# austintheriot/ray-tracer-webgl

Hardware: AMD Instinct MI355X
Metric: Mray/s (ray segments/s) at 1920x1080 (higher is better)
Workload: dtype f32

## Files before the change

ray_tracer_webgl_amd/csrc/pt_api.hip:

```cpp
#include <hip/hip_runtime.h>

#include <mutex>
#include <chrono>
#include <cmath>
#include <cstdarg>
#include <cstdio>
#include <cstdlib>
#include <cstring>
#include <new>
#include <string>
#include <thread>
#include <utility>
#include <vector>

#include "../../include/ptrace.h"
#include "../../include/ptrace_dev.h"
#include "pt_bvh.hpp"
#include "pt_grid.hpp"
#include "pt_grid_records.hpp"
#include "pt_scene_image.hpp"
#include "pt_extra.h"
#include "pt_sigs.h"
#include "pt_kernel_args.h"
#include "pt_geom_plan.hpp"
// ... 231 lines not shown
  }
  if (const ptbuf::Fit f = c->feat.fit(e); !f.ok()) return fit_refused(c, "feature planes", f, e);
  {
    if (c->query.on && !c->query.fits(e)) PT_HIP(c, hipStreamSynchronize(c->stream));
    const ptbuf::Fit f = c->query.fit(e);
    if (f.fresh & c->query.ORDER) PT_HIP(c, fill_identity_order(c->query.order, e.tiles));
    if (!f.ok()) return fit_refused(c, "query planes", f, e);
  }
  if (const ptbuf::Fit f = c->hist.fit(e); !f.ok()) return fit_refused(c, "history planes", f, e);
  {
    const ptbuf::Fit f = c->expo.fit();
    if (f.fresh & c->expo.STATE) PT_HIP(c, zero(c->expo.state, c->expo.kWords));
    if (!f.ok()) return fit_refused(c, "exposure state", f, e);
  }
  if (const ptbuf::Fit f = c->glare.fit(c->width, c->local_rows); !f.ok()) return fit_refused(c, "glare pyramid", f, e);
  return PT_OK;
}

int frame_buffers_ready(pt_ctx* c, const char* who) {
  const ptbuf::Extent e = extent_of(c);
  if (c->frame.in_place(e) && (!c->est.on || c->est.in_place(e, c->hist.on))) return PT_OK;
  return fail(c, PT_ERR_CAPACITY, "%s: the context's buffers are not allocated for the rows in place (an earlier allocation failed)", who);
}

enum OptInSet { SET_ESTIMATE, SET_FEATURES, SET_QUERIES, SET_REPROJECT, SET_TONEMAP, SET_GLARE, SET_NEXT_EVENT };
int option_off(pt_ctx* c, const char* who, OptInSet set, int code = PT_ERR_NOT_READY) {
  static const char* const what[] = {"the error estimate is off (pt_set_option PT_OPT_ERROR_ESTIMATE)", "the feature planes are off (pt_set_option PT_OPT_FEATURES)",
                                     "ray queries are off (pt_set_option PT_OPT_RAY_QUERIES)", "reprojection is off (pt_set_option PT_OPT_REPROJECT)",
                                     "tone mapping is off (pt_set_option PT_OPT_TONEMAP)", "the glare is off (pt_set_option PT_OPT_GLARE)",
                                     "next-event estimation is off (pt_set_option PT_OPT_NEXT_EVENT)"};
  return fail(c, code, "%s: %s", who, what[set]);
}

int clear_error(pt_ctx* c) {
  if (!c->est.on) return PT_OK;
  const size_t pix = n_pixels(c);
  if (pix) PT_HIP(c, hipMemsetAsync(c->est.state.get(), 0, 2 * pix * sizeof(float4), c->stream));
  c->est.spp = 0;
  return PT_OK;
}

int empty_accum(pt_ctx* c) {
  const size_t pix = n_pixels(c);
  if (c->frame.accum && pix) PT_HIP(c, hipMemsetAsync(c->frame.accum, 0, pix * sizeof(float4), c->stream));
  return clear_error(c);
}

int fold_events(pt_ctx* c) {
  for (size_t i = 0; i < c->events_used; i++) {
    float ms = 0.f;
    PT_HIP(c, hipEventElapsedTime(&ms, c->events[i].first, c->events[i].second));
    c->kernel_ms += (double)ms;
  }
  c->events_used = 0;
  return PT_OK;
}

int next_events(pt_ctx* c, std::pair<hipEvent_t, hipEvent_t>** ev) {
  if (c->events_used == c->events.size()) {
    if (c->events.size() >= 512) {
      PT_HIP(c, hipStreamSynchronize(c->stream));
      int rc = fold_events(c);
      if (rc != PT_OK) return rc;
    } else {
      hipEvent_t a, b;
      PT_HIP(c, hipEventCreate(&a));
      PT_HIP(c, hipEventCreate(&b));
      c->events.emplace_back(a, b);
    }
  }
  *ev = &c->events[c->events_used++];
  return PT_OK;
}

struct TimedSpan {
  std::pair<hipEvent_t, hipEvent_t>* ev = nullptr;
  int take(pt_ctx* c) { return next_events(c, &ev); }
  int begin(pt_ctx* c) const {
    if (ev) PT_HIP(c, hipEventRecord(ev->first, c->stream));
    return PT_OK;
  }
  int end(pt_ctx* c) const {
    if (ev) PT_HIP(c, hipEventRecord(ev->second, c->stream));
    return PT_OK;
  }
};

bool is_capturing(const pt_ctx* c) {
  hipStreamCaptureStatus cap = hipStreamCaptureStatusNone;
  (void)hipStreamIsCapturing(c->stream, &cap);
  return cap != hipStreamCaptureStatusNone;
}
int not_capturing(pt_ctx* c, const char* who) {
  return is_capturing(c) ? fail(c, PT_ERR_INVALID, "%s: synchronises; not inside a stream capture", who) : PT_OK;
}

int scene_and_uniforms(pt_ctx* c, const char* who) {
  if (c->state.have_spheres && c->state.have_params) return PT_OK;
  return fail(c, PT_ERR_NOT_READY, "%s: pt_set_spheres and pt_set_params must come first", who);
}

int launch_tile_order(pt_ctx* c) {
  hipLaunchKernelGGL(pt_tile_order_kernel, dim3(1), dim3(1024), 0, c->stream, c->frame.tile_cost.get(), c->frame.tile_order.get(),
                     n_tiles(c));
  PT_HIP(c, hipGetLastError());
  return PT_OK;
}

void try_finish_tuning(pt_ctx* c) {
  if (!c->geom.awaiting_times()) return;
  for (int k = 0; k < c->geom.n_paths; k++)
    if (hipEventQuery(c->trial_ev[2 * k + 1]) != hipSuccess) return;
  double ms[4];
  for (int k = 0; k < c->geom.n_paths; k++) {
    float t = 0.f;
    if (hipEventElapsedTime(&t, c->trial_ev[2 * k], c->trial_ev[2 * k + 1]) != hipSuccess) return;
    ms[k] = (double)t;
  }
  c->geom.settle(ms);
}

PathScene path_scene(const pt_ctx* c) {
  return {c->list.n, c->bvh.present, c->grid.present, c->grid.head.max_cell_entries, c->grid.head.n_always};
}

double need_factor(const pt_ctx* c) {
  return c->grid.present && c->state.have_params ? view_need_factor(c->params, c->grid.head.c0, c->grid.head.s0) : 0.0;
}

int fit_state(const pt_ctx* c) {
  return grid_fit_state(c->geom.grid_in_use(c->grid.present), need_factor(c), (double)c->grid.head.near_factor);
}

Staging grid_build(const pt_ctx* c) {
  const ptgrid::Grid& g = c->grid.head;
  return grid_staging(ptscene::staged_cells(g), g.n_entries, walk_lds_room(), c->state.grid_cells_build, fit_state(c));
}

const void* cell_kernel(int device, const TraceCell& k) {
#define PT_TRACE_ACCESSOR_OF(object, accessor, n_ids) accessor,
  static const void* (*const accessors[OBJ_COUNT + 2])(int) = {PT_TRACE_OBJECTS(PT_TRACE_ACCESSOR_OF) pt_nee_kernel, pt_rad_nee_kernel};
  static_assert(OBJ_NEE == OBJ_COUNT && OBJ_RAD_NEE == OBJ_COUNT + 1, "the next-event objects follow the trace table's");
  static std::once_flag once[64][OBJ_COUNT + 2][PT_EXTRA_COUNT];
  static_assert(PT_EXTRA_COUNT >= PT_VARIANT_COUNT, "the extra object has the most ids");
  const void* fn = accessors[k.object](k.id);
  if (fn && k.object >= OBJ_EXTRA)
    std::call_once(once[device & 63][k.object][k.id], [fn] {
      (void)hipFuncSetAttribute(fn, hipFuncAttributeMaxDynamicSharedMemorySize, (int)kWalkLdsMax);
      (void)hipGetLastError();
    });
  return fn;
}

}

PT_API int pt_device_count(void) {
  int n = 0;
  if (hipGetDeviceCount(&n) != hipSuccess) return 0;
  return n;
}

PT_API const char* pt_last_error(pt_ctx* ctx) {
  return ctx ? ctx->error.c_str() : g_create_error.c_str();
}

static int create_common(pt_ctx** out, int device, uint32_t width, uint32_t height, void* caller_stream) {
  if (!out) return fail(nullptr, PT_ERR_INVALID, "pt_create: out is NULL");
  *out = nullptr;
  if (width == 0 || height == 0) return fail(nullptr, PT_ERR_INVALID, "pt_create: empty image");
  int n = 0;
  const double t_begin = host_ms();
  if (hipGetDeviceCount(&n) != hipSuccess || n <= 0)
    return fail(nullptr, PT_ERR_NO_DEVICE,
                "pt_create: no HIP device (libptrace has no CPU backend by design)");
  const double t_runtime = host_ms();
  if (device < 0 || device >= n)
    return fail(nullptr, PT_ERR_NO_DEVICE, "pt_create: device %d out of range (0..%d)", device, n - 1);
  pt_ctx* c = new (std::nothrow) pt_ctx();
  if (!c) return fail(nullptr, PT_ERR_INVALID, "pt_create: out of host memory");
  c->device = device;
  c->width = width;
  c->height = height;
  c->local_rows = height;
  auto bail = [&](hipError_t e, const char* what) {
    fail(nullptr, PT_ERR_HIP, "pt_create: %s: %s", what, hipGetErrorString(e));
    delete c;
    return PT_ERR_HIP;
  };
  hipError_t e;
  if ((e = hipSetDevice(device)) != hipSuccess) return bail(e, "hipSetDevice");
  hipDeviceProp_t prop;
  if ((e = hipGetDeviceProperties(&prop, device)) != hipSuccess) return bail(e, "hipGetDeviceProperties");
  c->num_cus = prop.multiProcessorCount > 0 ? prop.multiProcessorCount : 256;
  const double t_device = host_ms();
  if (caller_stream) {
    c->stream = (hipStream_t)caller_stream;
  } else {
    if ((e = hipStreamCreateWithFlags(&c->own_stream, hipStreamNonBlocking)) != hipSuccess)
      return bail(e, "hipStreamCreateWithFlags");
    c->stream = c->own_stream;
  }
  const double t_stream = host_ms();
  if ((e = (hipError_t)c->d_counters.reserve(PT_CTR_ALLOC)) != hipSuccess) return bail(e, "hipMalloc(counters)");
  const double t_first_malloc = host_ms();
  if ((e = hipMemsetAsync(c->d_counters.get(), 0, PT_CTR_ALLOC * sizeof(unsigned long long), c->stream)) != hipSuccess)
    return bail(e, "hipMemsetAsync(counters)");
  const double t_first_memset = host_ms();
  if ((e = (hipError_t)c->d_frame_ctr.reserve(2)) != hipSuccess) return bail(e, "hipMalloc(frame counter)");
  if ((e = hipMemsetAsync(c->d_frame_ctr.get(), 0, 2 * sizeof(uint32_t), c->stream)) != hipSuccess)
    return bail(e, "hipMemsetAsync(frame counter)");
  const double t_small_allocs = host_ms();
  for (int id = 0; id < PT_MAIN_COUNT; id++) (void)hipFuncSetAttribute(pt_main_kernel(id), hipFuncAttributeMaxDynamicSharedMemorySize, (int)kWalkLdsMax);
  (void)hipGetLastError();
  const double t_code = host_ms();
  int rc = ensure_buffers(c);
  if (rc != PT_OK) { g_create_error = c->error; delete c; return rc; }
  const double t_end = host_ms();
  c->setup_ms[PT_SETUP_CREATE_RUNTIME] = t_runtime - t_begin;
  c->setup_ms[PT_SETUP_CREATE_DEVICE] = t_device - t_runtime;
  c->setup_ms[PT_SETUP_CREATE_STREAM_ALLOCS] = t_small_allocs - t_device;
  c->setup_ms[PT_SETUP_CREATE_STREAM] = t_stream - t_device;
  c->setup_ms[PT_SETUP_CREATE_FIRST_MALLOC] = t_first_malloc - t_stream;
  c->setup_ms[PT_SETUP_CREATE_FIRST_MEMSET] = t_first_memset - t_first_malloc;
  c->setup_ms[PT_SETUP_CREATE_CODE_OBJECT] = t_code - t_small_allocs;
  c->setup_ms[PT_SETUP_CREATE_BUFFERS] = t_end - t_code;
  c->setup_ms[PT_SETUP_CREATE_TOTAL] = t_end - t_begin;
  *out = c;
  return PT_OK;
}

PT_API int pt_create(pt_ctx** out, int device, uint32_t width, uint32_t height) {
  return create_common(out, device, width, height, nullptr);
}
PT_API int pt_create_on_stream(pt_ctx** out, int device, uint32_t width, uint32_t height, void* hip_stream) {
  return create_common(out, device, width, height, hip_stream);
}

PT_API int pt_destroy(pt_ctx* c) {
  if (!c) return PT_ERR_INVALID;
  (void)hipSetDevice(c->device);
  (void)hipStreamSynchronize(c->stream);
  delete c;
  return PT_OK;
}

PT_API int pt_set_stream(pt_ctx* c, void* hip_stream) {
  if (!c) return PT_ERR_INVALID;
  PT_HIP(c, hipSetDevice(c->device));
  PT_HIP(c, hipStreamSynchronize(c->stream));
  int rc = fold_events(c);
  if (rc != PT_OK) return rc;
  if (!hip_stream && !c->own_stream)
    PT_HIP(c, hipStreamCreateWithFlags(&c->own_stream, hipStreamNonBlocking));
  c->stream = hip_stream ? (hipStream_t)hip_stream : c->own_stream;
  return PT_OK;
}

namespace {

#define PT_TRY(call) do { if (int rc_ = (call); rc_ != PT_OK) return rc_; } while (0)

template <class T>
int upload(pt_ctx* c, DevBuf<T>& buf, const T* src, size_t n, size_t n_pad, int pad_byte) {
  if (buf.capacity() < n_pad) PT_HIP(c, buf.reserve(n_pad));
  if (n_pad > n) PT_HIP(c, hipMemset(buf.get() + n, pad_byte, (n_pad - n) * sizeof(T)));
  if (n) PT_HIP(c, hipMemcpy(buf.get(), src, n * sizeof(T), hipMemcpyHostToDevice));
  return PT_OK;
}
template <class T>
int upload(pt_ctx* c, DevBuf<T>& buf, const std::vector<T>& src) { return upload(c, buf, src.data(), src.size(), src.size(), 0); }
template <class T>
void release(std::vector<T>& v) { std::vector<T>().swap(v); }

void drop_scene(pt_ctx* c) {
  c->bvh.present = c->grid.present = false;
  changed(*c, ptstate::SCENE_DROPPED);
}

int install_list(pt_ctx* c, const ptscene::Split& sp, size_t n) {
  PT_TRY(upload(c, c->list.geom, sp.geom));
  PT_TRY(upload(c, c->list.mat, sp.mat.data(), n, n ? n : 1u, 0));
  return upload(c, c->list.r0, sp.r0.data(), 2 * n, n ? 2 * n : 2u, 0);
}

int install_slots(pt_ctx* c, SceneSlots& s, const std::vector<uint32_t>& index, size_t n, size_t n_pad, const ptscene::Split& sp) {
  s.present = false;
  PT_TRY(upload(c, s.index, index.data(), n, n_pad, 0xff));
  s.index_n = n_pad;
  return upload(c, s.mat, ptscene::per_slot(index.data(), n, sp.mat.data(), sp.mat.size()).data(), n, n_pad, 0);
}

int install_bvh(pt_ctx* c, ptbvh::Bvh& bvh, const ptscene::Split& sp) {
  PT_TRY(install_slots(c, c->bvh, bvh.slot_index, bvh.slot_index.size(), bvh.slot_index.size(), sp));
  PT_TRY(upload(c, c->bvh.nodes, bvh.nodes16));
  PT_TRY(upload(c, c->bvh.nodes32, bvh.nodes32));
  PT_TRY(upload(c, c->bvh.slots, bvh.slots));
  release(bvh.nodes); release(bvh.nodes16); release(bvh.nodes32); release(bvh.slots); release(bvh.slot_index);
  c->bvh.head = std::move(bvh);
  c->bvh.present = true;
  return PT_OK;
}
int install_grid(pt_ctx* c, ptgrid::Grid& grid, const ptscene::Split& sp) {
  const size_t n_ent = grid.n_entries, n_ent_pad = n_ent + 4u;
  PT_TRY(install_slots(c, c->grid, grid.entry_index, n_ent, n_ent_pad, sp));
  PT_TRY(upload(c, c->grid.entries, grid.entries.data(), n_ent * 4, n_ent_pad * 4, 0));
  std::vector<uint32_t> recs(grid.cells.size());
  for (size_t k = 0; k < recs.size(); k++) recs[k] = ptrec::from_host(grid.cells[k]);
  PT_TRY(upload(c, c->grid.cells, recs.data(), recs.size(), (recs.size() + 3u) & ~(size_t)3u, 0));
  if (grid.n[1] == 1u) {
    recs.assign(((size_t)ptrec::ring_cells(grid.n[0], grid.n[2]) + 3u) & ~(size_t)3u, ptrec::kOutside);
    ptrec::ring_layout(grid.cells.data(), grid.n[0], grid.n[2], recs.data());
    PT_TRY(upload(c, c->grid.ring, recs));
  }
  release(grid.cells); release(grid.entries); release(grid.entry_index);
  c->grid.head = std::move(grid);
  c->grid.present = true;
  return PT_OK;
}

inline bool wants_uuids(const pt_ctx* c) { return c->dbg_enable || c->feat.on || c->query.on; }
int upload_uuids(pt_ctx* c, const std::vector<int32_t>& uuid) {
  PT_HIP(c, hipSetDevice(c->device));
  PT_HIP(c, hipStreamSynchronize(c->stream));
  PT_TRY(upload(c, c->list.uuid, uuid.data(), uuid.size(), uuid.empty() ? 1u : uuid.size(), 0));
  for (SceneSlots* s : std::initializer_list<SceneSlots*>{&c->bvh, &c->grid}) {
    if (!s->present || !s->index_n) continue;
    std::vector<uint32_t> index(s->index_n);
    PT_HIP(c, hipMemcpy(index.data(), s->index.get(), index.size() * sizeof(uint32_t), hipMemcpyDeviceToHost));
    PT_TRY(upload(c, s->uuid, ptscene::per_slot(index.data(), index.size(), uuid.data(), uuid.size())));
  }
  changed(*c, ptstate::UUIDS_UPLOADED);
  return PT_OK;
}

int upload_lights(pt_ctx* c, const ptscene::Split& sp, uint32_t n) {
  std::vector<ptnee::Light> table(n ? n : 1u);
  const uint32_t L = ptnee::lights_of(sp.geom.data(), sp.mat.data(), n, table.data());
  const ptbuf::Fit f = c->lights.fit(L);
  if (!f.ok()) return fail(c, PT_ERR_HIP, "PT_OPT_NEXT_EVENT: no room for the table of %u lights (%s)", L, hipGetErrorString((hipError_t)f.err));
  if (L) PT_HIP(c, hipMemcpy(c->lights.table.get(), table.data(), (size_t)L * sizeof(ptnee::Light), hipMemcpyHostToDevice));
  return PT_OK;
}

int install_scene(pt_ctx* c, const ptscene::Split& sp, uint32_t n, ptbvh::Bvh* bvh, ptgrid::Grid* grid) {
  PT_TRY(install_list(c, sp, n));
  if (bvh) PT_TRY(install_bvh(c, *bvh, sp));
  if (grid) PT_TRY(install_grid(c, *grid, sp));
  if (c->lights.on) PT_TRY(upload_lights(c, sp, n));
  return wants_uuids(c) ? upload_uuids(c, sp.uuid) : PT_OK;
}

}

PT_API int pt_set_spheres(pt_ctx* c, const PtSphere* s, uint32_t n) {
  if (!c || (!s && n)) return fail(c, PT_ERR_INVALID, "pt_set_spheres: NULL argument");
  if (n > PT_MAX_SPHERES)
    return fail(c, PT_ERR_CAPACITY, "pt_set_spheres: %u spheres exceed the 16-bit candidate index range (%u)",
                n, PT_MAX_SPHERES);
  PT_HIP(c, hipSetDevice(c->device));
  const double t_begin = host_ms();
  ptscene::Split sp = ptscene::split(s, n);
  const double t_split = host_ms();
  ptbvh::Bvh bvh;
  const bool have_bvh = sp.regular && ptbvh::build(sp.geom.data(), sp.radii.data(), n, &bvh);
  const double t_bvh = host_ms();
  ptgrid::Grid grid;
  const bool have_grid = sp.regular && ptscene::build_grid(sp.geom.data(), sp.radii.data(), n, 3.0, &grid);
  const double t_grid = host_ms();
  PT_HIP(c, hipStreamSynchronize(c->stream));
  drop_scene(c);
  if (int rc = install_scene(c, sp, n, have_bvh ? &bvh : nullptr, have_grid ? &grid : nullptr); rc != PT_OK) return drop_scene(c), rc;
  c->list.n = n;
  c->list.host = std::move(sp);
  changed(*c, ptstate::SCENE_INSTALLED);
  c->geom.reset();
  c->geom.list_paths(path_scene(c));
  const double t_end = host_ms();
  c->setup_ms[PT_SETUP_SPHERES_SPLIT] = t_split - t_begin;
  c->setup_ms[PT_SETUP_SPHERES_BVH_BUILD] = t_bvh - t_split;
  c->setup_ms[PT_SETUP_SPHERES_GRID_BUILD] = t_grid - t_bvh;
  c->setup_ms[PT_SETUP_SPHERES_UPLOAD] = t_end - t_grid;
  c->setup_ms[PT_SETUP_SPHERES_TOTAL] = t_end - t_begin;
  return PT_OK;
}

PT_API int pt_set_params(pt_ctx* c, const PtParams* p) {
  if (!c || !p) return fail(c, PT_ERR_INVALID, "pt_set_params: NULL argument");
  if (p->width != c->width || p->height != c->height)
    return fail(c, PT_ERR_INVALID, "pt_set_params: %ux%u does not match the context's %ux%u (use pt_resize)",
                p->width, p->height, c->width, c->height);
  if (p->samples_per_pixel < 1 || p->max_depth < 1)
    return fail(c, PT_ERR_INVALID, "pt_set_params: samples_per_pixel and max_depth must be >= 1");
  if (p->band_count > 1 && (p->band_rows == 0 || p->band_index >= p->band_count))
    return fail(c, PT_ERR_INVALID, "pt_set_params: bad row partition (rows %u index %u count %u)",
                p->band_rows, p->band_index, p->band_count);
  PT_HIP(c, hipSetDevice(c->device));
  uint32_t rows = count_local_rows(c->height, *p);
  const bool repartition = rows != c->local_rows || ptstate::Partition(*p) != ptstate::Partition(c->params);
  if (repartition && c->frame.accum_bound && (size_t)rows * c->width > c->frame.accum_pixels)
    return fail(c, PT_ERR_CAPACITY, "pt_set_params: bound accumulation buffer too small for %u rows", rows);
  if (repartition) {
    changed(*c, ptstate::ROWS_ASKED);
    const uint32_t old_rows = c->local_rows;
    c->local_rows = rows;
    int rc = ensure_buffers(c);
    if (rc != PT_OK) {
      c->local_rows = old_rows;
      return rc;
    }
    c->params = *p;
    changed(*c, ptstate::UNIFORMS_OTHER_ROWS);
    c->tally.repartitioned();
    if (int rc = empty_accum(c); rc != PT_OK) return rc;
    return pt_clear_textures(c);
  }
  c->params = *p;
  changed(*c, ptstate::UNIFORMS_SAME_ROWS);
  return PT_OK;
}

PT_API int pt_resize(pt_ctx* c, uint32_t width, uint32_t height) {
  if (!c || width == 0 || height == 0) return fail(c, PT_ERR_INVALID, "pt_resize: bad size");
  PT_HIP(c, hipSetDevice(c->device));
  PT_HIP(c, hipStreamSynchronize(c->stream));
  c->width = width;
  c->height = height;
  changed(*c, ptstate::RESIZED);
  c->params.band_count = 0;
  c->local_rows = height;
  if (c->frame.accum_bound) { c->frame.accum_bound = false; c->frame.accum = nullptr; }
  int rc = ensure_buffers(c);
  if (rc != PT_OK) return rc;
  rc = pt_clear_textures(c);
  if (rc != PT_OK) return rc;
  return pt_reset_accum(c);
}

PT_API int pt_reserve_passes(pt_ctx* c, uint32_t max_passes) {
  if (!c || max_passes == 0) return fail(c, PT_ERR_INVALID, "pt_reserve_passes: bad argument");
  PT_HIP(c, hipSetDevice(c->device));
  const double t_begin = host_ms();
  const uint32_t reserved = c->reserved_passes;
  if (max_passes > reserved) {
    PT_HIP(c, hipStreamSynchronize(c->stream));
    c->reserved_passes = max_passes;
  }
  const int rc = ensure_buffers(c);
  if (rc != PT_OK) c->reserved_passes = reserved;
  c->setup_ms[PT_SETUP_RESERVE_TOTAL] = host_ms() - t_begin;
  return rc;
}

PT_API int pt_reset_accum(pt_ctx* c) {
  if (!c) return PT_ERR_INVALID;
  PT_HIP(c, hipSetDevice(c->device));
  PT_HIP(c, hipMemsetAsync(c->d_counters.get(), 0, PT_CTR_COUNT * sizeof(unsigned long long), c->stream));
  if (int rc = empty_accum(c); rc != PT_OK) return rc;
  PT_HIP(c, hipStreamSynchronize(c->stream));
  c->events_used = 0;
  c->kernel_ms = 0.0;
  c->tally.emptied();
  return PT_OK;
}

PT_API int pt_bind_accum(pt_ctx* c, void* dev_ptr, size_t bytes) {
  if (!c) return PT_ERR_INVALID;
  PT_HIP(c, hipSetDevice(c->device));
  PT_HIP(c, hipStreamSynchronize(c->stream));
  if (!dev_ptr) {
    c->frame.accum_bound = false;
    c->frame.accum = nullptr;
    c->tally.rebound();
    if (int rc = ensure_buffers(c); rc != PT_OK) return rc;
    return empty_accum(c);
  }
  size_t need = n_pixels(c) * sizeof(float4);
  if (bytes < need) return fail(c, PT_ERR_CAPACITY, "pt_bind_accum: %zu bytes < %zu needed", bytes, need);
  if (((uintptr_t)dev_ptr & 15u) != 0) return fail(c, PT_ERR_INVALID, "pt_bind_accum: pointer not 16-byte aligned");
  c->frame.accum = (float4*)dev_ptr;
  c->frame.accum_pixels = bytes / sizeof(float4);
  c->frame.accum_bound = true;
  c->tally.rebound();
  return clear_error(c);
}

PT_API int pt_accum_ptr(pt_ctx* c, void** dev_ptr, size_t* bytes) {
  if (!c || !dev_ptr) return PT_ERR_INVALID;
  *dev_ptr = c->frame.accum;
  if (bytes) *bytes = n_pixels(c) * sizeof(float4);
  return PT_OK;
}

PT_API int pt_read_accum(pt_ctx* c, float* dst, size_t bytes) {
  if (!c || !dst) return fail(c, PT_ERR_INVALID, "pt_read_accum: NULL argument");
  const size_t need = n_pixels(c) * sizeof(float4);
  if (bytes < need) return fail(c, PT_ERR_CAPACITY, "pt_read_accum: %zu bytes < %zu needed", bytes, need);
  PT_HIP(c, hipSetDevice(c->device));
  if (need) PT_HIP(c, hipMemcpyAsync(dst, c->frame.accum, need, hipMemcpyDefault, c->stream));
  PT_HIP(c, hipStreamSynchronize(c->stream));
  return PT_OK;
}

PT_API int pt_load_accum(pt_ctx* c, const float* src, size_t bytes) {
  if (!c || !src) return fail(c, PT_ERR_INVALID, "pt_load_accum: NULL argument");
  const size_t need = n_pixels(c) * sizeof(float4);
  if (bytes != need)
    return fail(c, PT_ERR_INVALID, "pt_load_accum: %zu bytes, the current row partition holds %zu", bytes, need);
  if (int rc = frame_buffers_ready(c, "pt_load_accum"); rc != PT_OK) return rc;
  PT_HIP(c, hipSetDevice(c->device));
  if (need == 0) return PT_OK;
  const size_t n_pix = n_pixels(c);
  PT_HIP(c, hipMemcpyAsync(c->frame.resolve.get(), src, need, hipMemcpyDefault, c->stream));
  float4 ends[2];
  PT_HIP(c, hipMemcpyAsync(&ends[0], c->frame.resolve.get(), sizeof(float4), hipMemcpyDeviceToHost, c->stream));
  PT_HIP(c, hipMemcpyAsync(&ends[1], c->frame.resolve.get() + (n_pix - 1), sizeof(float4), hipMemcpyDeviceToHost, c->stream));
  PT_HIP(c, hipStreamSynchronize(c->stream));
  const float w = ends[0].w;
  if (!(w >= 0.0f) || w >= 16777216.0f || w != std::floor(w))
    return fail(c, PT_ERR_INVALID, "pt_load_accum: sample count %g in the buffer is not a count", (double)w);
  if (ends[1].w != w)
    return fail(c, PT_ERR_INVALID, "pt_load_accum: sample counts differ across the buffer (%g ... %g): not an accumulation of whole passes",
                (double)w, (double)ends[1].w);
  PT_HIP(c, hipMemcpyAsync(c->frame.accum, c->frame.resolve.get(), need, hipMemcpyDeviceToDevice, c->stream));
  if (int rc = clear_error(c); rc != PT_OK) return rc;
  PT_HIP(c, hipStreamSynchronize(c->stream));
  c->tally.loaded((uint32_t)w, n_pix);
  return PT_OK;
}

static int fill_uniforms(pt_ctx* c, uint32_t n_passes, PtKernelArgs& A) {
  const PtParams& p = c->params;
  memset(&A, 0, sizeof A);
  for (int k = 0; k < 3; k++) {
    A.origin[k] = p.camera_origin[k];
    A.horizontal[k] = p.horizontal[k];
    A.vertical[k] = p.vertical[k];
    A.llc[k] = p.lower_left_corner[k];
    A.cam_u[k] = p.u[k];
    A.cam_v[k] = p.v[k];
  }
  A.lens_radius = p.lens_radius;
  {
    bool off = p.lens_radius == 0.0f;
    for (int k = 0; k < 3; k++) {
      off = off && std::isfinite(p.u[k]) && std::isfinite(p.v[k]);
      off = off && !(p.camera_origin[k] == 0.0f && std::signbit(p.camera_origin[k]));
    }
    A.lens_off = off ? 1u : 0u;
  }
  A.time0 = p.time;
  A.time_step = p.time_step != 0.0f ? p.time_step : 1.0f;
  A.first_pass = p.first_pass;
  A.spp = p.samples_per_pixel;
  A.max_depth = p.max_depth;
  A.rr_min_depth = c->rr_min_depth;
  A.background_mode = p.background_mode;
  A.width = c->width;
  A.height = c->height;
  A.local_rows = c->local_rows;
  A.band_rows = p.band_rows ? p.band_rows : 1;
  A.band_index = p.band_index;
  A.band_count = p.band_count;
  A.n_passes = n_passes;
  A.n_spheres = c->list.n;
  A.scene_regular = c->list.host.regular ? 1u : 0u;
  A.tiles_x = tiles_x(c);
  A.tiles_y = tiles_y(c);
  unsigned long long items = (unsigned long long)A.tiles_x * A.tiles_y * n_passes * 64ull;
  if (items > 0xfffffff0ull)
    return fail(c, PT_ERR_CAPACITY, "pt_render_passes: %llu work items exceed 2^32; render fewer passes per call", items);
  A.n_items = (uint32_t)items;
  A.fw = (float)c->width;
  A.fh = (float)c->height;
  A.div_per_tile = pt_div_make(64u * n_passes);
  A.div_tiles_x = pt_div_make(A.tiles_x);
  A.div_band_rows = pt_div_make(A.band_rows);
  A.geom = c->list.geom.get();
  A.mat = c->list.mat.get();
  A.mat_r0 = c->list.r0.get();
  A.slab = reinterpret_cast<float*>(c->frame.slab.get());
  A.counters = c->d_counters.get();
  A.tile_order = c->frame.tile_order.get();
  A.tile_cost = c->frame.tile_cost.get();
  A.carry_lanes = c->carry_lanes;
  A.refill_min = c->refill_min;
  A.frame_ctr = c->d_frame_ctr.get() + 1;
  if (c->dbg_enable) {
    A.uuid = c->list.uuid.get();
    A.dbg_selected = c->dbg_selected;
    for (int k = 0; k < 3; k++) A.dbg_cursor[k] = c->dbg_cursor[k];
  }
  return PT_OK;
}

static Staging bind_hierarchy(pt_ctx* c, PtKernelArgs& A) {
  const SceneBvh& b = c->bvh;
  A.bvh_nodes = b.nodes.get();
  A.bvh_nodes32 = b.nodes32.get();
  A.bvh_slots = b.slots.get();
  A.bvh_slot_index = b.index.get();
  A.slot_mat = b.mat.get();
  if (c->dbg_enable) A.slot_uuid = b.uuid.get();
  A.n_nodes = b.head.n_nodes;
  A.n_tree_slots = b.head.n_tree_slots;
  A.n_slots = b.head.n_slots;
  A.n_outliers = b.head.n_outliers;
// ... 1792 lines not shown
```

ray_tracer_webgl_amd/csrc/pt_grid_records.hpp:

```cpp
#pragma once
#include <cstdint>

#if defined(__HIPCC__)
#define PT_REC_FN __host__ __device__ inline
#else
#define PT_REC_FN inline
#endif

namespace ptrec {

constexpr uint32_t kFirstBits = 23;
constexpr uint32_t kFirstMask = (1u << kFirstBits) - 1u;
constexpr uint32_t kNone = 1u << kFirstBits;
constexpr uint32_t kLong = 256u;
constexpr uint32_t kEntryLimit = (1u << kFirstBits) - 8u;
PT_REC_FN bool fits(uint32_t n_entries) { return n_entries < kEntryLimit; }

PT_REC_FN uint32_t field_of(uint32_t count) { return count <= 4u ? (1u << count) - 1u : (kLong | count); }
PT_REC_FN uint32_t encode(uint32_t first, uint32_t count) { return first | (field_of(count) << kFirstBits); }
PT_REC_FN uint32_t from_host(uint32_t host_rec) { return encode(host_rec & 0xffffffu, host_rec >> 24); }

PT_REC_FN uint32_t first_of(uint32_t rec) { return rec & kFirstMask; }
PT_REC_FN bool is_long(uint32_t rec) { return (int32_t)rec < 0; }
PT_REC_FN uint32_t count_of(uint32_t rec) {
  const uint32_t f = rec >> kFirstBits;
  if (f & kLong) return f & 255u;
  return (f & 1u) + ((f >> 1) & 1u) + ((f >> 2) & 1u) + ((f >> 3) & 1u);
}
PT_REC_FN uint32_t to_host(uint32_t rec) { return first_of(rec) | (count_of(rec) << 24); }

PT_REC_FN uint32_t round_mask(uint32_t rec, uint32_t G) {
  const uint32_t all = (1u << G) - 1u;
  return is_long(rec) ? all : ((rec >> kFirstBits) & all);
}
PT_REC_FN uint32_t next(uint32_t rec, uint32_t G) {
  const uint32_t left = count_of(rec);
  return left > G ? encode(first_of(rec) + G, left - G) : 0u;
}
PT_REC_FN uint32_t short_mask4(uint32_t rec, uint32_t cand) { return cand & (rec >> kFirstBits); }
PT_REC_FN uint32_t next_long4(uint32_t rec) { return encode(first_of(rec) + 4u, ((rec >> kFirstBits) & 255u) - 4u); }

constexpr uint32_t kOutside = 0u;
constexpr uint32_t kRing2 = 2u;
PT_REC_FN uint64_t ring_cells(uint32_t nx, uint32_t nz) { return (uint64_t)(nx + kRing2) * (nz + kRing2); }
PT_REC_FN uint32_t ring_index(uint32_t nx, uint32_t cx, uint32_t cz) { return (cz + 1u) * (nx + kRing2) + (cx + 1u); }
PT_REC_FN uint32_t ring_record(uint32_t host_rec) {
  const uint32_t rec = from_host(host_rec);
  return rec == kOutside ? 1u : rec;
}
inline void ring_layout(const uint32_t* host_cells, uint32_t nx, uint32_t nz, uint32_t* out) {
  const uint64_t n = ring_cells(nx, nz);
  for (uint64_t k = 0; k < n; k++) out[k] = kOutside;
  for (uint32_t cz = 0; cz < nz; cz++)
    for (uint32_t cx = 0; cx < nx; cx++) out[ring_index(nx, cx, cz)] = ring_record(host_cells[(uint64_t)cz * nx + cx]);
}

}
```

ray_tracer_webgl_amd/csrc/pt_grid_walk.hpp:

```cpp
#pragma once
#include "pt_grid_records.hpp"
#include "pt_scene.hpp"

namespace ptk {

template <typename S, bool COUNT>
__device__ __forceinline__ void grid_walk(const PtKernelArgs& A, const Path& p, bool scan_lane, int n_live, Carry& cw,
                                          GridWalk& w, Hit& h, Tally<COUNT>& tally) {
  karg_t& K = *kargs();
  const V3 o = p.o; const V3 d = p.d; const float a = p.a;
  float closest = h.closest; int hit = h.hit; uint32_t lit_from = h.lit_from;
  bool carried = cw.carried; uint32_t hit_pos = cw.hit_pos;
  float tmx = w.tmx, tmy = w.tmy, tmz = w.tmz, t_exit = w.t_exit;
  uint32_t cell = w.cell, rem = w.rem, pend = w.pend;
  const uint32_t n_cell_entries = A.n_tree_slots;
  const bool fresh = scan_lane && !carried;
  const float ya = rcp_newton(a);
  const uint32_t a_guard = hit_root_guard(a);

  auto exact_group = [&](uint32_t base, uint32_t& mask, float hb0, float hb1, float hb2, float hb3, float ds0, float ds1,
                         float ds2, float ds3) {
    for (unsigned long long m_x = pt_ballot(mask != 0u); m_x != 0ull; m_x = pt_ballot(mask != 0u)) {
      tally.exact(m_x);
      if (mask != 0u) {
        const uint32_t k = first_candidate(mask);
        mask &= mask - 1u;
        const float half_b = k == 0u ? hb0 : (k == 1u ? hb1 : (k == 2u ? hb2 : hb3));
        const float disc = k == 0u ? ds0 : (k == 1u ? ds1 : (k == 2u ? ds2 : ds3));
        const float v = hit_root(half_b, disc, a, ya, a_guard);
        const uint32_t pos = base + k;
        bool wins = v < closest;
        if (v == closest)
          wins = hit_pos == 0xffffffffu || A.bvh_slot_index[pos] > A.bvh_slot_index[hit_pos];
        if (!(v < PT_MIN_T) && wins) {
          closest = v;
          hit_pos = pos;
        }
      }
    }
  };
  auto pass_bit = [](float hb, float cc, float ds) -> uint32_t { return ((f2u(cc) | f2u(hb)) & ~f2u(ds + 0.0f)) >> 31; };

  tally.always_group(true);
  if (S::WALK != 4 && A.n_outliers == 1u) {
    const uint32_t base = n_cell_entries;
    float4 e0;
    if constexpr (S::WALK == 4) { e0 = S::slot_at(A, base); }
    else { const f4v s0 = S::c_slots(A)[base]; e0 = make_float4(s0.x, s0.y, s0.z, s0.w); }
    float hb0, cc0, ds0; sphere_test(o, d, a, e0, hb0, cc0, ds0);
    const bool cand = fresh && pass_bit(hb0, cc0, ds0) != 0u;
    if (pt_ballot(cand) != 0ull) {
      tally.exact(pt_ballot(cand));
      if (cand) {
        const float v = hit_root(hb0, ds0, a, ya, a_guard);
        if (!(v < PT_MIN_T) && v <= closest) {
          closest = v;
          hit_pos = base;
        }
      }
    }
  } else {
    const uint32_t n_grp = (A.n_outliers + 3u) >> 2;
    for (uint32_t gi = 0; gi < n_grp; gi++) {
      const uint32_t base = n_cell_entries + 4u * gi;
      float4 e0, e1, e2, e3;
      if constexpr (S::WALK == 4) {
        e0 = S::slot_at(A, base); e1 = S::slot_at(A, base + 1u); e2 = S::slot_at(A, base + 2u); e3 = S::slot_at(A, base + 3u);
      } else {
        const f4v s0 = S::c_slots(A)[base], s1 = S::c_slots(A)[base + 1u], s2 = S::c_slots(A)[base + 2u], s3 = S::c_slots(A)[base + 3u];
        e0 = make_float4(s0.x, s0.y, s0.z, s0.w); e1 = make_float4(s1.x, s1.y, s1.z, s1.w);
        e2 = make_float4(s2.x, s2.y, s2.z, s2.w); e3 = make_float4(s3.x, s3.y, s3.z, s3.w);
      }
      float hb0, cc0, ds0; sphere_test(o, d, a, e0, hb0, cc0, ds0);
      float hb1, cc1, ds1; sphere_test(o, d, a, e1, hb1, cc1, ds1);
      float hb2, cc2, ds2; sphere_test(o, d, a, e2, hb2, cc2, ds2);
      float hb3, cc3, ds3; sphere_test(o, d, a, e3, hb3, cc3, ds3);
      uint32_t mask = pass_bit(hb0, cc0, ds0) | (pass_bit(hb1, cc1, ds1) << 1) | (pass_bit(hb2, cc2, ds2) << 2) | (pass_bit(hb3, cc3, ds3) << 3);
      mask = fresh ? mask : 0u;
      exact_group(base, mask, hb0, hb1, hb2, hb3, ds0, ds1, ds2, ds3);
    }
  }
  tally.always_group(false);
  tally.phase(2);
  const float ix = __builtin_amdgcn_fmed3f(__builtin_amdgcn_rcpf(d.x), -1e18f, 1e18f);
  const float iy = __builtin_amdgcn_fmed3f(__builtin_amdgcn_rcpf(d.y), -1e18f, 1e18f);
  const float iz = __builtin_amdgcn_fmed3f(__builtin_amdgcn_rcpf(d.z), -1e18f, 1e18f);
  const bool posx = ix > 0.0f, posy = iy > 0.0f, posz = iz > 0.0f;
  const float tdx = K.grid_h[0] * __builtin_fabsf(ix), tdz = K.grid_h[2] * __builtin_fabsf(iz);
  const int gnx = (int)K.grid_n[0], gnz = (int)K.grid_n[2];
  const int sdx = posx ? 1 : -1;
  float tdy = 0.0f;
  int gny = 1, sdy = 0;
  if constexpr (!S::FLAT_Y) {
    tdy = K.grid_h[1] * __builtin_fabsf(iy);
    gny = (int)K.grid_n[1];
    sdy = posy ? gnx : -gnx;
  }
  const int row = S::FLAT_Y ? gnx + (int)ptrec::kRing2 : gnx;
  const int sdz = posz ? row * gny : -(row * gny);

  if (!carried) { rem = 0u; pend = 0u; }
  if constexpr (S::FLAT_Y) { if (!carried) cell = 0u; }
  if (pt_ballot(fresh) != 0ull) {
    if (fresh) tally.flag(PT_REG_WALK_ENTRY);
    const float px = o.x - K.bvh_c0[0], py = o.y - K.bvh_c0[1], pz = o.z - K.bvh_c0[2];
    const float r2 = fma_(pz, pz, fma_(py, py, px * px));
    const bool near = r2 <= K.grid_r2_near;
    float mm = 0.0f;
    if (pt_ballot(fresh && !near) != 0ull)
      mm = near ? 0.0f : 1.7e-3f * (__builtin_amdgcn_sqrtf(r2) + K.bvh_s0);
    const float oix = o.x * ix, oiy = o.y * iy, oiz = o.z * iz;
    const float t1x = fma_(K.grid_lo_n[0] - mm, ix, -oix), t2x = fma_(K.grid_hi_n[0] + mm, ix, -oix);
    const float t1y = fma_(K.grid_lo_n[1] - mm, iy, -oiy), t2y = fma_(K.grid_hi_n[1] + mm, iy, -oiy);
    const float t1z = fma_(K.grid_lo_n[2] - mm, iz, -oiz), t2z = fma_(K.grid_hi_n[2] + mm, iz, -oiz);
    const float tn = __builtin_fmaxf(
        __builtin_fmaxf(__builtin_fminf(t1x, t2x), __builtin_fminf(t1y, t2y)),
        __builtin_fmaxf(__builtin_fminf(t1z, t2z), 0.0f));
    const float tf = __builtin_fminf(
        __builtin_fminf(__builtin_fmaxf(t1x, t2x), __builtin_fmaxf(t1y, t2y)),
        __builtin_fmaxf(t1z, t2z));
    bool enter = fresh && tn <= __builtin_fminf(tf, closest);
    if (enter && !near) {
      tally.flag(PT_REG_WALK_FAR_RAY);
      atomicAdd(&A.counters[PT_CTR_FAR_RAYS], 1ull);
      lit_from = 0u;
      closest = PT_MAX_T;
      hit_pos = 0xffffffffu;
      enter = false;
    }
    if constexpr (S::FLAT_Y) {
      if (enter) {
        tally.flag(PT_REG_WALK_ENTER_CELL);
        const float glx = K.grid_lo[0], glz = K.grid_lo[2];
        const float ghx = K.grid_h[0], ghz = K.grid_h[2];
        const float fx = (fma_(d.x, tn, o.x) - glx) * K.grid_inv_h[0];
        const float fz = (fma_(d.z, tn, o.z) - glz) * K.grid_inv_h[2];
        const int nx1 = gnx - 1, nz1 = gnz - 1;
        int cx = (int)__builtin_floorf(fx), cz = (int)__builtin_floorf(fz);
        cx = cx < 0 ? 0 : (cx > nx1 ? nx1 : cx);
        cz = cz < 0 ? 0 : (cz > nz1 ? nz1 : cz);
        const float bx = fma_((float)(cx + (posx ? 1 : 0)), ghx, glx);
        const float bz = fma_((float)(cz + (posz ? 1 : 0)), ghz, glz);
        tmx = __builtin_fmaxf(fma_(bx, ix, -oix), tn);
        tmy = __builtin_fmaxf(t1y, t2y);
        tmz = __builtin_fmaxf(fma_(bz, iz, -oiz), tn);
        cell = (uint32_t)(cz + 1) * (uint32_t)row + (uint32_t)(cx + 1);
      }
    } else
    if (enter) {
      tally.flag(PT_REG_WALK_ENTER_CELL);
      const float glx = K.grid_lo[0], gly = K.grid_lo[1], glz = K.grid_lo[2];
      const float ghx = K.grid_h[0], ghy = K.grid_h[1], ghz = K.grid_h[2];
      const float fx = (fma_(d.x, tn, o.x) - glx) * K.grid_inv_h[0];
      const float fy = (fma_(d.y, tn, o.y) - gly) * K.grid_inv_h[1];
      const float fz = (fma_(d.z, tn, o.z) - glz) * K.grid_inv_h[2];
      const int nx1 = gnx - 1, ny1 = gny - 1, nz1 = gnz - 1;
      int cx = (int)__builtin_floorf(fx), cy = (int)__builtin_floorf(fy), cz = (int)__builtin_floorf(fz);
      cx = cx < 0 ? 0 : (cx > nx1 ? nx1 : cx);
      cy = cy < 0 ? 0 : (cy > ny1 ? ny1 : cy);
      cz = cz < 0 ? 0 : (cz > nz1 ? nz1 : cz);
      const float bx = fma_((float)(cx + (posx ? 1 : 0)), ghx, glx);
      const float by = fma_((float)(cy + (posy ? 1 : 0)), ghy, gly);
      const float bz = fma_((float)(cz + (posz ? 1 : 0)), ghz, glz);
      tmx = __builtin_fmaxf(fma_(bx, ix, -oix), tn);
      tmy = __builtin_fmaxf(fma_(by, iy, -oiy), tn);
      tmz = __builtin_fmaxf(fma_(bz, iz, -oiz), tn);
      rem = (uint32_t)((posx ? nx1 - cx : cx) + 1) | ((uint32_t)((posy ? ny1 - cy : cy) + 1) << 10) |
            ((uint32_t)((posz ? nz1 - cz : cz) + 1) << 20);
      cell = ((uint32_t)cz * (uint32_t)gny + (uint32_t)cy) * (uint32_t)gnx + (uint32_t)cx;
    }
  }

  tally.phase(3);
  auto on = [&]() -> bool { if constexpr (S::FLAT_Y) return cell != 0u; else return rem != 0u; };
  uint32_t walk_iters = 0;
  const uint32_t carry_base = A.carry_lanes, carry_slope = A.carry_lanes != 0u ? 4u : 0u;
  const uint32_t half_live = ((uint32_t)n_live + 1u) >> 1;
  for (;;) {
    unsigned long long m_mv = pt_ballot(on()) & pt_ballot(pend < ptrec::kNone);
#define PT_CELL_STEP_FLAT \
        tally.walk(m_mv); \
        if (cell != 0u && pend < ptrec::kNone) { \
          const uint32_t rec = S::cell_at(A, cell); \
          const float tmin = __builtin_fminf(__builtin_fminf(tmx, tmy), tmz); \
          const bool isx = tmx == tmin; \
          const bool endy = !isx && tmy == tmin; \
          t_exit = tmin; \
          pend = rec; \
          tmx += isx ? tdx : 0.0f; \
          tmz += isx ? 0.0f : tdz; \
          cell += (uint32_t)(isx ? sdx : sdz); \
          cell = (rec == ptrec::kOutside || endy || (rec < ptrec::kNone && closest < tmin)) ? 0u : cell; \
        }
#define PT_CELL_STEP_XYZ \
        tally.walk(m_mv); \
        if (rem != 0u && pend < ptrec::kNone) { \
          const uint32_t rec = S::cell_at(A, cell); \
          const float tmin = __builtin_fminf(__builtin_fminf(tmx, tmy), tmz); \
          const bool isx = tmx == tmin; \
          const bool isy = !isx && tmy == tmin; \
          const bool isz = !isx && !isy; \
          t_exit = tmin; \
          pend = rec; \
          tmx += isx ? tdx : 0.0f; \
          tmy += isy ? tdy : 0.0f; \
          tmz += isz ? tdz : 0.0f; \
          const uint32_t dec = isx ? 1u : (isy ? 1024u : 1048576u); \
          rem -= dec; \
          const bool out = (rem & (dec * 1023u)) == 0u; \
          cell += (uint32_t)(isx ? sdx : (isy ? sdy : sdz)); \
          rem = (out || (rec < ptrec::kNone && closest < tmin)) ? 0u : rem; \
        }
#define PT_CELL_STEP \
        if constexpr (S::FLAT_Y) { PT_CELL_STEP_FLAT } else { PT_CELL_STEP_XYZ }
    if (m_mv != 0ull) {
      tally.walk_first();
      PT_CELL_STEP
      m_mv = pt_ballot(on()) & pt_ballot(pend < ptrec::kNone);
      while (__builtin_expect(m_mv != 0ull, 0)) {
        PT_CELL_STEP
        m_mv = pt_ballot(on()) & pt_ballot(pend < ptrec::kNone);
      }
    }
#undef PT_CELL_STEP
#undef PT_CELL_STEP_FLAT
#undef PT_CELL_STEP_XYZ
    tally.phase(4);
    const bool has = pend >= ptrec::kNone;
    const unsigned long long m_has = pt_ballot(has);
    if (m_has == 0ull) break;
    tally.leaf(m_has);
    {
      constexpr uint32_t G = S::WALK == 4 ? 4u : (uint32_t)PT_LEAF_GROUP_GMEM;
      static_assert(G >= 2u && G <= 4u, "a leaf round tests two, three or four entries");
      const uint32_t base = pend & ptrec::kFirstMask;
      tally.leaf_cells(A, has, base, A.n_slots);
      float4 g[4];
#pragma unroll
      for (uint32_t k = 0; k < G; k++) g[k] = S::slot_at(A, base + k);
      float hb[4], cc[4], ds[4];
#pragma unroll
      for (uint32_t k = 0; k < G; k++) sphere_test(o, d, a, g[k], hb[k], cc[k], ds[k]);
#pragma unroll
      for (uint32_t k = G; k < 4u; k++) { hb[k] = hb[G - 1u]; ds[k] = ds[G - 1u]; }
      uint32_t cand = 0u;
#pragma unroll
      for (uint32_t k = 0; k < G; k++) cand |= pass_bit(hb[k], cc[k], ds[k]) << k;
      uint32_t mask;
      if constexpr (G == 4u) {
        mask = ptrec::short_mask4(pend, cand);
        const bool lng = ptrec::is_long(pend);
        const uint32_t rec = pend;
        pend = 0u;
        if (pt_ballot(lng) != 0ull) {
          if (lng) { mask = cand; pend = ptrec::next_long4(rec); }
        }
      } else {
        mask = cand & ptrec::round_mask(pend, G);
        pend = ptrec::next(pend, G);
      }
      exact_group(base, mask, hb[0], hb[1], hb[2], hb[3], ds[0], ds[1], ds[2], ds[3]);
      if constexpr (S::FLAT_Y) cell = (has && pend < ptrec::kNone && closest < t_exit) ? 0u : cell;
      else rem = (has && pend < ptrec::kNone && closest < t_exit) ? 0u : rem;
    }
    tally.phase(5);
    walk_iters++;
    const uint32_t n_on = (uint32_t)__popcll(pt_ballot(on()) | pt_ballot(pend >= ptrec::kNone));
    const int t = (int)walk_iters - 2;
    const uint32_t thr = t >= 0 ? carry_base + carry_slope * (uint32_t)t : 0u;
    const uint32_t lim = thr < half_live ? thr : half_live;
    if (n_on < (lim > 1u ? lim : 1u)) break;
  }
  carried = on() || pend >= ptrec::kNone;
  tally.carried(carried);
  if (hit_pos != 0xffffffffu) hit = 0;
  h.closest = closest; h.hit = hit; h.lit_from = lit_from;
  cw.carried = carried; cw.hit_pos = hit_pos;
  w.tmx = tmx; w.tmy = tmy; w.tmz = tmz; w.t_exit = t_exit;
  w.cell = cell; w.rem = rem; w.pend = pend;
}

}
```

ray_tracer_webgl_amd/csrc/pt_kernel_args.h:

```cpp
#pragma once
#include <stdint.h>

struct PtMatRec {
  float albedo[3];
  float fuzz;
  float refraction_index;
  int32_t type;
  float radius;
  float inv_ri;
};
static_assert(sizeof(PtMatRec) == 32, "PtMatRec must be 32 bytes");
struct PtDiv {
  uint32_t m, s1, s2;
};
static inline PtDiv pt_div_make(uint32_t d) {
  PtDiv r;
  uint32_t l = 0;
  while (l < 32 && (1ull << l) < (unsigned long long)d) l++;
  r.m = (uint32_t)(((1ull << 32) * ((1ull << l) - d)) / d + 1ull);
  r.s1 = l < 1 ? l : 1;
  r.s2 = l > 0 ? l - 1 : 0;
  return r;
}

struct PtKernelArgs {
  float origin[3], horizontal[3], vertical[3], llc[3], cam_u[3], cam_v[3];
  float lens_radius;
  float time0, time_step;
  uint32_t first_pass;
  int32_t spp;
  int32_t max_depth;
  int32_t background_mode;
  uint32_t width, height;
  uint32_t local_rows;
  uint32_t band_rows, band_index, band_count;
  uint32_t n_passes;
  uint32_t n_spheres;
  uint32_t scene_regular;
  uint32_t tiles_x, tiles_y;
  uint32_t n_items;
  const float* geom;
  const PtMatRec* mat;
  float* slab;
  unsigned long long* counters;
  const uint32_t* tile_order;
  uint32_t* tile_cost;
  const uint32_t* bvh_nodes;
  const float* bvh_nodes32;
  const float* bvh_slots;
  const uint32_t* bvh_slot_index;
  const PtMatRec* slot_mat;
  uint32_t n_nodes, n_tree_slots, n_slots, n_outliers;
  float bvh_c0[3], bvh_s0;
  const uint32_t* grid_cells;
  uint32_t n_cells;
  uint32_t grid_n[3];
  float grid_lo[3], grid_hi[3], grid_h[3], grid_inv_h[3];
  float grid_r2_near;
  float grid_lo_n[3], grid_hi_n[3];
  uint32_t lds_scene_bytes;
  unsigned long long* wave_log;
  uint32_t refill_min;
  uint32_t carry_lanes;
  float bvh_kinv;
  uint32_t block_threads;
  uint32_t queue_chunk;
  float fw, fh;
  PtDiv div_per_tile, div_tiles_x, div_band_rows;
  uint32_t coop_max_live;
  int32_t rr_min_depth;
  uint32_t lens_off;
  uint32_t queue_groups;
  uint32_t queue_static;
  uint32_t n_waves;
  uint32_t cost_feedback;
  uint32_t* cell_hist;
  const uint32_t* frame_ctr;
  const float* mat_r0;
  const int32_t* uuid;
  const int32_t* slot_uuid;
  float dbg_cursor[3];
  int32_t dbg_selected;
  uint32_t refill_ahead;
};

#ifndef PT_WAVES_WALK
#define PT_WAVES_WALK 6
#endif
#ifndef PT_WAVES_LIST
#define PT_WAVES_LIST 7
#endif
#define PT_WAVES_LIST_LDS 6
#ifndef PT_WAVES_SMALL
#define PT_WAVES_SMALL 7
#endif
#define PT_WAVES_TWIN_CELLS 4
#define PT_BUILT_FOR(n) __attribute__((amdgpu_waves_per_eu(n, n)))
#ifndef PT_LEAF_GROUP_GMEM
#define PT_LEAF_GROUP_GMEM 4
#endif

enum { PT_WAVE_LOG_WORDS = 4 };
enum { PT_COH_BINS = 66, PT_HIST_WAVE_STRIDE = 8 };
enum { PT_REG_REFILL_DECODE = 0, PT_REG_REFILL_RESERVE, PT_REG_CAMERA_RAY, PT_REG_SHADE_HIT_RECORD, PT_REG_SHADE_SKY, PT_REG_SHADE_DIFFUSE,
       PT_REG_SHADE_METAL, PT_REG_SHADE_GLASS, PT_REG_SHADE_GLASS_REFRACT, PT_REG_SHADE_CONTINUES, PT_REG_SHADE_FINISHED, PT_REG_SHADE_ITEM_STORE,
       PT_REG_WALK_ENTRY, PT_REG_WALK_ENTER_CELL, PT_REG_WALK_FAR_RAY, PT_REG_SHADE_ANY,
       PT_REG_REFILL_PROMOTE , PT_N_REGIONS };
enum { PT_CTR_HEAD = 0, PT_CTR_SEGMENTS = 1, PT_CTR_SAMPLES = 2, PT_CTR_FAR_RAYS = 3 , PT_CTR_REGIONS_MORE = 4 , PT_CTR_SCRATCH = 7 , PT_CTR_WORK = 8, PT_CTR_LITERAL = 16, PT_CTR_PHASES = 24, PT_N_PHASES = 8, PT_CTR_REGIONS = 32, PT_CTR_TIMEBINS = 64, PT_CTR_COUNT = 128,
       PT_QUEUE_GROUPS_MAX = 256, PT_CTR_GROUP_HEADS = 128 ,
       PT_CTR_ALLOC = PT_CTR_GROUP_HEADS + 8 * PT_QUEUE_GROUPS_MAX };

#define PT_LDS_ENTRIES(n) ((((n) + 7u) & ~7u) + 4u)
#define PT_MAX_SPHERES_SMALL 16u
#define PT_MAX_SPHERES_LDS 10232u
#define PT_PARK_DWORDS 14u
#ifndef PT_PARK_STRIDE
#define PT_PARK_STRIDE 15u
#endif
#define PT_BVH_LDS_BYTES32(n_nodes, n_slots) ((((size_t)(n_nodes) + 1u) * 2u + (size_t)(n_slots)) * 16u)
#define PT_BVH_LDS_BYTES16(n_nodes) (((size_t)(n_nodes) + 1u) * 16u)
#define PT_GRID_LDS_CELLS(n_cells) ((((size_t)(n_cells) + 3u) / 4u) * 16u)
#define PT_MAX_SPHERES 65528u

enum {
  PT_PROBE_HASH = 0,
  PT_PROBE_SINCOS = 1,
  PT_PROBE_CBRT = 2,
  PT_PROBE_UNIT_SPHERE = 3,
  PT_PROBE_DIVSQRT = 4,
  PT_PROBE_BASE_HASH = 5,
  PT_PROBE_FAST_ARITH = 6,
};
```

Measured before the change: 61420.

## Test the widest always-tested sphere first, then the rest in groups of three

```diff
diff --git a/ray_tracer_webgl_amd/csrc/pt_api.hip b/ray_tracer_webgl_amd/csrc/pt_api.hip
--- a/ray_tracer_webgl_amd/csrc/pt_api.hip
+++ b/ray_tracer_webgl_amd/csrc/pt_api.hip
@@ -557,6 +557,7 @@
 }
 int install_grid(pt_ctx* c, ptgrid::Grid& grid, const ptscene::Split& sp) {
   const size_t n_ent = grid.n_entries, n_ent_pad = n_ent + 4u;
+  ptrec::lead_to_front(grid.entries.data(), grid.entry_index.data(), grid.n_cell_entries, grid.n_always, grid.c0);
   PT_TRY(install_slots(c, c->grid, grid.entry_index, n_ent, n_ent_pad, sp));
   PT_TRY(upload(c, c->grid.entries, grid.entries.data(), n_ent * 4, n_ent_pad * 4, 0));
   std::vector<uint32_t> recs(grid.cells.size());
diff --git a/ray_tracer_webgl_amd/csrc/pt_grid_records.hpp b/ray_tracer_webgl_amd/csrc/pt_grid_records.hpp
--- a/ray_tracer_webgl_amd/csrc/pt_grid_records.hpp
+++ b/ray_tracer_webgl_amd/csrc/pt_grid_records.hpp
@@ -1,4 +1,6 @@
 #pragma once
+#include <cmath>
+#include <cstddef>
 #include <cstdint>
 
 #if defined(__HIPCC__)
@@ -55,4 +57,32 @@
     for (uint32_t cx = 0; cx < nx; cx++) out[ring_index(nx, cx, cz)] = ring_record(host_cells[(uint64_t)cz * nx + cx]);
 }
 
+inline uint32_t lead_of(const float* group, uint32_t n_always, const float* c0) {
+  uint32_t lead = 0;
+  double best = -1.0;
+  for (uint32_t k = 0; k < n_always; k++) {
+    const double dx = (double)group[4 * k] - c0[0], dy = (double)group[4 * k + 1] - c0[1], dz = (double)group[4 * k + 2] - c0[2];
+    const double reach = std::sqrt(dx * dx + dy * dy + dz * dz) + std::sqrt((double)group[4 * k + 3]);
+    if (reach > best) { best = reach; lead = k; }
+  }
+  return lead;
 }
+inline void lead_first(float* group, uint32_t* index, uint32_t lead) {
+  const float e[4] = {group[4 * lead], group[4 * lead + 1], group[4 * lead + 2], group[4 * lead + 3]};
+  const uint32_t ix = index[lead];
+  for (uint32_t k = lead; k > 0; k--) {
+    for (int j = 0; j < 4; j++) group[4 * k + j] = group[4 * (k - 1) + j];
+    index[k] = index[k - 1];
+  }
+  for (int j = 0; j < 4; j++) group[j] = e[j];
+  index[0] = ix;
+}
+inline uint32_t lead_to_front(float* entries, uint32_t* index, uint32_t n_cell_entries, uint32_t n_always, const float* c0) {
+  if (n_always == 0u) return 0u;
+  float* group = entries + 4 * (size_t)n_cell_entries;
+  const uint32_t lead = lead_of(group, n_always, c0);
+  lead_first(group, index + n_cell_entries, lead);
+  return lead;
+}
+
+}
diff --git a/ray_tracer_webgl_amd/csrc/pt_grid_walk.hpp b/ray_tracer_webgl_amd/csrc/pt_grid_walk.hpp
--- a/ray_tracer_webgl_amd/csrc/pt_grid_walk.hpp
+++ b/ray_tracer_webgl_amd/csrc/pt_grid_walk.hpp
@@ -41,43 +41,45 @@
   };
   auto pass_bit = [](float hb, float cc, float ds) -> uint32_t { return ((f2u(cc) | f2u(hb)) & ~f2u(ds + 0.0f)) >> 31; };
 
+  auto always_slot = [&](uint32_t pos) -> float4 {
+    if constexpr (S::WALK == 4) { return S::slot_at(A, pos); }
+    else { const f4v s = S::c_slots(A)[pos]; return make_float4(s.x, s.y, s.z, s.w); }
+  };
   tally.always_group(true);
-  if (S::WALK != 4 && A.n_outliers == 1u) {
-    const uint32_t base = n_cell_entries;
-    float4 e0;
-    if constexpr (S::WALK == 4) { e0 = S::slot_at(A, base); }
-    else { const f4v s0 = S::c_slots(A)[base]; e0 = make_float4(s0.x, s0.y, s0.z, s0.w); }
-    float hb0, cc0, ds0; sphere_test(o, d, a, e0, hb0, cc0, ds0);
-    const bool cand = fresh && pass_bit(hb0, cc0, ds0) != 0u;
+  const uint32_t n_always = A.n_outliers;
+  {
+    const bool lead_on = fresh && n_always != 0u;
+    float hb0, cc0, ds0; sphere_test(o, d, a, always_slot(n_cell_entries), hb0, cc0, ds0);
+    const bool cand = lead_on && pass_bit(hb0, cc0, ds0) != 0u;
     if (pt_ballot(cand) != 0ull) {
       tally.exact(pt_ballot(cand));
       if (cand) {
         const float v = hit_root(hb0, ds0, a, ya, a_guard);
         if (!(v < PT_MIN_T) && v <= closest) {
           closest = v;
-          hit_pos = base;
-        }
-      }
-    }
-  } else {
-    const uint32_t n_grp = (A.n_outliers + 3u) >> 2;
-    for (uint32_t gi = 0; gi < n_grp; gi++) {
-      const uint32_t base = n_cell_entries + 4u * gi;
-      float4 e0, e1, e2, e3;
-      if constexpr (S::WALK == 4) {
-        e0 = S::slot_at(A, base); e1 = S::slot_at(A, base + 1u); e2 = S::slot_at(A, base + 2u); e3 = S::slot_at(A, base + 3u);
-      } else {
-        const f4v s0 = S::c_slots(A)[base], s1 = S::c_slots(A)[base + 1u], s2 = S::c_slots(A)[base + 2u], s3 = S::c_slots(A)[base + 3u];
-        e0 = make_float4(s0.x, s0.y, s0.z, s0.w); e1 = make_float4(s1.x, s1.y, s1.z, s1.w);
-        e2 = make_float4(s2.x, s2.y, s2.z, s2.w); e3 = make_float4(s3.x, s3.y, s3.z, s3.w);
-      }
-      float hb0, cc0, ds0; sphere_test(o, d, a, e0, hb0, cc0, ds0);
-      float hb1, cc1, ds1; sphere_test(o, d, a, e1, hb1, cc1, ds1);
-      float hb2, cc2, ds2; sphere_test(o, d, a, e2, hb2, cc2, ds2);
-      float hb3, cc3, ds3; sphere_test(o, d, a, e3, hb3, cc3, ds3);
-      uint32_t mask = pass_bit(hb0, cc0, ds0) | (pass_bit(hb1, cc1, ds1) << 1) | (pass_bit(hb2, cc2, ds2) << 2) | (pass_bit(hb3, cc3, ds3) << 3);
-      mask = fresh ? mask : 0u;
-      exact_group(base, mask, hb0, hb1, hb2, hb3, ds0, ds1, ds2, ds3);
+          hit_pos = n_cell_entries;
+        }
+      }
+    }
+  }
+  {
+    constexpr uint32_t GA = (uint32_t)PT_ALWAYS_GROUP;
+    static_assert(GA >= 2u && GA <= 4u, "a round of the always-tested group tests two, three or four entries");
+    const uint32_t n_others = n_always - (n_always != 0u ? 1u : 0u);
+    for (uint32_t first = 0; first < n_others; first += GA) {
+      const uint32_t base = n_cell_entries + 1u + first;
+      const uint32_t left = n_others - first;
+      const uint32_t valid = left >= GA ? (1u << GA) - 1u : (1u << left) - 1u;
+      float hb[4], cc[4], ds[4];
+#pragma unroll
+      for (uint32_t k = 0; k < GA; k++) sphere_test(o, d, a, always_slot(base + k), hb[k], cc[k], ds[k]);
+#pragma unroll
+      for (uint32_t k = GA; k < 4u; k++) { hb[k] = hb[GA - 1u]; ds[k] = ds[GA - 1u]; }
+      uint32_t mask = 0u;
+#pragma unroll
+      for (uint32_t k = 0; k < GA; k++) mask |= pass_bit(hb[k], cc[k], ds[k]) << k;
+      mask = fresh ? (mask & valid) : 0u;
+      exact_group(base, mask, hb[0], hb[1], hb[2], hb[3], ds[0], ds[1], ds[2], ds[3]);
     }
   }
   tally.always_group(false);
diff --git a/ray_tracer_webgl_amd/csrc/pt_kernel_args.h b/ray_tracer_webgl_amd/csrc/pt_kernel_args.h
--- a/ray_tracer_webgl_amd/csrc/pt_kernel_args.h
+++ b/ray_tracer_webgl_amd/csrc/pt_kernel_args.h
@@ -99,6 +99,9 @@
 #ifndef PT_LEAF_GROUP_GMEM
 #define PT_LEAF_GROUP_GMEM 4
 #endif
+#ifndef PT_ALWAYS_GROUP
+#define PT_ALWAYS_GROUP 3
+#endif
 
 enum { PT_WAVE_LOG_WORDS = 4 };
 enum { PT_COH_BINS = 66, PT_HIST_WAVE_STRIDE = 8 };
```

Result: no change. 61590, median of 6 (+0.3%).
